# xxayt/MGSV

Hardware: AMD Instinct MI355X
Metric: video-music pairs/s fwd+bwd at B=64 (full training step); sub-objects: retrieval sim-matrix GB/s, eval forward pairs/s (higher is better)
Workload: dtype bf16; 1 GPU; BASELINE.json configs[2]: B=64/GPU, T_v=30, T_a=512, D=512, train mode (dropout on), f32 master weights + Adam, f32 gradient accumulation; global_batch=64, launch=tape

## Files before the change

mgsv_amd/csrc/linear.hip:

```cpp
#include "common.h"

namespace {

constexpr int BM = 128, BN = 128;
constexpr int KB = 128;
constexpr int LDS_ROW = KB + 16;
constexpr int NTHREADS = 256;

template <typename TC> struct Frag;
template <> struct Frag<float>  { typedef f32x4  type; };
template <> struct Frag<bf16_t> { typedef bf16x8 type; };

template <typename TC>
__device__ __forceinline__ typename Frag<TC>::type zero_frag() {
    typename Frag<TC>::type z;
#pragma unroll
    for (int i = 0; i < elem_traits<TC>::per16; ++i) z[i] = (TC)0.f;
    return z;
}

template <typename TA, typename TC>
__device__ __forceinline__ typename Frag<TC>::type load_a_frag(const TA* __restrict__ p, const TA* __restrict__ p2) {
    constexpr int n = elem_traits<TC>::per16;
    float v[n];
// ... 339 lines not shown
                SplitF32x4 sa[2][2], sw2[2][2];
#pragma unroll
                for (int u = 0; u < 2; ++u)
#pragma unroll
                    for (int t = 0; t < 2; ++t) {
                        sa[u][t] = made_split4(*(const f32x4*)(la + t * 32 * LDS_ROW + (ks + u) * 32));
                        sw2[u][t] = made_split4(*(const f32x4*)(lw + t * 32 * LDS_ROW + (ks + u) * 32));
                    }
#pragma unroll
                for (int mt = 0; mt < 2; ++mt)
#pragma unroll
                    for (int nt = 0; nt < 2; ++nt)
                        acc[mt][nt] = transposed ? made_mfma_x3_16(sw2[0][nt], sw2[1][nt], sa[0][mt], sa[1][mt], acc[mt][nt])
                                                 : made_mfma_x3_16(sa[0][mt], sa[1][mt], sw2[0][nt], sw2[1][nt], acc[mt][nt]);
            }
        } else {
#pragma unroll
        for (int ks = 0; ks < 4; ++ks) {
            frag_t fa[2], fw[2];
#pragma unroll
            for (int t = 0; t < 2; ++t) {
                fa[t] = *(const frag_t*)(la + t * 32 * LDS_ROW + ks * 32);
                fw[t] = *(const frag_t*)(lw + t * 32 * LDS_ROW + ks * 32);
            }
#pragma unroll
            for (int mt = 0; mt < 2; ++mt)
#pragma unroll
                for (int nt = 0; nt < 2; ++nt) {
                    if constexpr (sizeof(TC) == 2) {
                        if (transposed)
                            acc[mt][nt] = __builtin_amdgcn_mfma_f32_32x32x16_bf16(fw[nt], fa[mt], acc[mt][nt], 0, 0, 0);
                        else
                            acc[mt][nt] = __builtin_amdgcn_mfma_f32_32x32x16_bf16(fa[mt], fw[nt], acc[mt][nt], 0, 0, 0);
                    } else {
#pragma unroll
                        for (int e = 0; e < 4; ++e) {
                            if (transposed)
                                acc[mt][nt] = __builtin_amdgcn_mfma_f32_32x32x2f32(fw[nt][e], fa[mt][e], acc[mt][nt], 0, 0, 0);
                            else
                                acc[mt][nt] = __builtin_amdgcn_mfma_f32_32x32x2f32(fa[mt][e], fw[nt][e], acc[mt][nt], 0, 0, 0);
                        }
                    }
                }
        }
        }
        if (kt + 1 < nk) store_stage(lds + ((kt + 1) & 1) * STAGE);
        __syncthreads();
    }

    float* Ct = (float*)lds;
#pragma unroll
    for (int mt = 0; mt < 2; ++mt)
#pragma unroll
        for (int nt = 0; nt < 2; ++nt)
#pragma unroll
            for (int e = 0; e < 16; ++e) {
                int row, col;
                if (transposed) { row = wn * 64 + nt * 32 + acc_row(e, hh); col = wm * 64 + mt * 32 + r; }
                else            { row = wm * 64 + mt * 32 + acc_row(e, hh); col = wn * 64 + nt * 32 + r; }
                Ct[row * CT_LD + col] = acc[mt][nt][e];
            }
    __syncthreads();

    if (splitk > 1) {
        float* wsp = a.split_ws + (int64_t)blockIdx.z * M * N;
        const int cc = tid & 15;
        const int n = n0 + cc * 8;
        const bool vec = (N % 4 == 0);
        for (int i = 0; i < 8; ++i) {
            const int row = (tid >> 4) + 16 * i;
            const int m = m0 + row;
            if (m >= M) break;
            const float* cp = Ct + row * CT_LD + cc * 8;
            if (vec && n + 8 <= N) {
                *(f32x4*)(wsp + (int64_t)m * N + n) = *(const f32x4*)cp;
                *(f32x4*)(wsp + (int64_t)m * N + n + 4) = *(const f32x4*)(cp + 4);
            } else {
                for (int j = 0; j < 8 && n + j < N; ++j) wsp[(int64_t)m * N + n + j] = cp[j];
            }
        }
        return;
    }
    unsigned char* outp = (unsigned char*)seg.out;
    const int64_t out_z = z * seg.out_z_stride;
    const int rpb = (int)seg.rows_per_batch, rmod = (int)a.r_row_mod;
    const int colb = (int)seg.col_begin;
    const int odt = seg.out_dtype;

    if (!transposed) {
        const int cc = tid & 15;
        const int n = n0 + cc * 8;
        int nvalid = N - n; nvalid = nvalid > 8 ? 8 : nvalid;
        if (nvalid > 0) {
            float bv[8];
            load_bias8(a.bias, n, N, bv);
            const bool out_vec = (seg.ldo % 8 == 0) && (seg.out_batch_stride % 8 == 0) && (seg.out_z_stride % 8 == 0) &&
                                 (((uintptr_t)outp & 15) == 0) && (colb % 8 == 0);
            const bool r_vec = a.R && (a.ldr % 8 == 0) && (((uintptr_t)a.R & 15) == 0);
#pragma unroll 2
            for (int i = 0; i < 8; ++i) {
                const int row = (tid >> 4) + 16 * i;
                const int ml = m0 + row;
                if (ml >= Mv) break;
                const int m = a.row_index ? a.row_index[ml] : ml;
                const float* cp = Ct + row * CT_LD + cc * 8;
                f32x4 c0 = *(const f32x4*)cp, c1 = *(const f32x4*)(cp + 4);
                float v[8] = {c0[0], c0[1], c0[2], c0[3], c1[0], c1[1], c1[2], c1[3]};
                epilogue8<true>(a, m, n, nvalid, v, bv, rmod, r_vec);
                int64_t orow;
                if (rpb > 0) {
                    const int b = m / rpb, t = m - b * rpb;
                    orow = (int64_t)b * seg.out_batch_stride + (int64_t)t * seg.ldo;
                } else {
                    orow = (int64_t)m * seg.ldo;
                }
                store8(outp, odt, out_z + orow + (n - colb), v, nvalid, out_vec);
            }
        }
    } else {
        const int col = tid & 127;
        const int m = m0 + col;
        if (m < M) {
            int64_t obase;
            if (rpb > 0) {
                const int b = m / rpb, t = m - b * rpb;
                obase = (int64_t)b * seg.out_batch_stride + t;
            } else {
                obase = m;
            }
            const bool zero = a.out_row_mask != nullptr && a.out_row_mask[m] == 0.f;
            const int rr = rmod > 0 ? m % rmod : m;
            for (int i = 0; i < 64; ++i) {
                const int row = (tid >> 7) + 2 * i;
                const int n = n0 + row;
                if (n >= N) break;
                float v = Ct[row * CT_LD + col];
                if (a.bias) v += a.bias[n];
                v = apply_act(v, a.act);
                if (a.R) v += load_as_f32(a.R, a.r_dtype, (int64_t)rr * a.ldr + n);
                if (zero) v = 0.f;
                store_from_f32(outp, odt, out_z + obase + (int64_t)(n - colb) * seg.ldo, v);
            }
        }
    }
}



constexpr int G_CT_LD = BN + 4;

__device__ __forceinline__ int swz(int row) { return (row >> 1) & 7; }

template <int NST, bool TRAIN, int BMT, typename TC = bf16_t, bool X3 = false>
__global__ __launch_bounds__(NTHREADS, NST == 1 ? (BMT == 64 ? 6 : (TRAIN ? 3 : 4)) : 1) void linear_glds_kernel(const MadeLinearArgs a) {
    constexpr int PER16 = 16 / (int)sizeof(TC), KE = KB / (int)sizeof(TC);
    constexpr int STAGE = (BMT + BN) * KB;
    constexpr int NT = BMT == 128 ? 2 : 1;
    constexpr int AP = BMT / 32;
    constexpr int EROWS = BMT == 128 ? 64 : 32;
    constexpr int CT_BYTES = EROWS * G_CT_LD * 4;
    __shared__ __attribute__((aligned(16))) unsigned char lds[NST == 1 ? (CT_BYTES > STAGE ? CT_BYTES : STAGE) : NST * STAGE];
    const int tid = threadIdx.x;
    const int lane = tid & 63, wave = tid >> 6;
    const int r = lane & 31, hh = lane >> 5;
    const int wm = BMT == 128 ? wave >> 1 : 0, wn = BMT == 128 ? wave & 1 : wave;

    const int M = (int)a.M, N = (int)a.N, K = (int)a.K;
    const int n_tiles = (N + BN - 1) / BN;
    int Mv = M;
    if (a.n_rows) { const int nv = *a.n_rows; Mv = nv < M ? nv : M; }
    const int nwg = ((Mv + BMT - 1) / BMT) * n_tiles;
    if ((int)blockIdx.x >= nwg) return;
    int tile_id;
    {
        const int xcd = blockIdx.x & 7, q = nwg >> 3, rem = nwg & 7;
        tile_id = (xcd < rem ? xcd * (q + 1) : rem * (q + 1) + (xcd - rem) * q) + (blockIdx.x >> 3);
    }
    const int tile_m = tile_id / n_tiles, tile_n = tile_id % n_tiles;
    const int m0 = tile_m * BMT, n0 = tile_n * BN;
    const int64_t z = blockIdx.z;

    int si = 0;
#pragma unroll
    for (int s = 1; s < 4; ++s)
        if (s < a.nseg && n0 >= a.seg[s].col_begin) si = s;
    const MadeLinearSeg seg = a.seg[si];


    if (a.tile_skip_mask) {
        const int g0 = m0 + lane, g1 = m0 + 64 + lane;
        const float v0 = g0 < M ? a.tile_skip_mask[g0] : 0.f, v1 = (BMT == 128 && g1 < M) ? a.tile_skip_mask[g1] : 0.f;
        if (!__any(v0 != 0.f || v1 != 0.f)) {
            if (a.out_row_mask && !seg.transposed && (a.split_k <= 1)) {
                const int rpb0 = (int)seg.rows_per_batch;
                for (int idx = tid; idx < BMT * (BN / 8); idx += NTHREADS) {
                    const int row = idx / (BN / 8), c8 = idx % (BN / 8);
                    const int m = m0 + row, n = n0 + c8 * 8;
                    if (m >= M || n >= N) continue;
                    int64_t orow;
                    if (rpb0 > 0) { const int b = m / rpb0, t = m - b * rpb0; orow = (int64_t)b * seg.out_batch_stride + (int64_t)t * seg.ldo; }
                    else orow = (int64_t)m * seg.ldo;
                    const float zero8[8] = {0.f, 0.f, 0.f, 0.f, 0.f, 0.f, 0.f, 0.f};
                    int nv = N - n; nv = nv > 8 ? 8 : nv;
                    store8(seg.out, seg.out_dtype, blockIdx.z * seg.out_z_stride + orow + (n - (int)seg.col_begin), zero8, nv, false);
                }
            }
            return;
        }
    }

    const TC* Abase = ((seg.use_a2 && a.A2 && a.a2_replace) ? (const TC*)a.A2 : (const TC*)a.A) + z * a.a_z_stride;
    const int64_t lda = (seg.use_a2 && a.A2 && a.a2_replace) ? a.lda2 : a.lda;
    const TC* Wbase = (const TC*)a.W + z * a.w_z_stride;
    const TC* pa[AP];
    const TC* pw[4];
#pragma unroll
    for (int i = 0; i < AP; ++i) {
        const int row = 8 * (AP * wave + i) + (lane >> 3);
        const int chunk = (lane & 7) ^ swz(row);
        int gm = m0 + row; gm = gm < Mv ? gm : Mv - 1;
        if (a.row_index) gm = a.row_index[gm];
        pa[i] = Abase + (int64_t)gm * lda + chunk * PER16;
    }
#pragma unroll
    for (int i = 0; i < 4; ++i) {
        const int row = 8 * (4 * wave + i) + (lane >> 3);
        const int chunk = (lane & 7) ^ swz(row);
        int gn = n0 + row; gn = gn < N ? gn : N - 1;
        pw[i] = Wbase + (int64_t)gn * a.ldw + chunk * PER16;
    }
    typedef __attribute__((address_space(3))) void* lds_ptr_t;
    typedef const __attribute__((address_space(1))) void* glb_ptr_t;

    f32x16 acc[2][NT];
#pragma unroll
    for (int i = 0; i < 2; ++i)
#pragma unroll
        for (int j = 0; j < NT; ++j)
#pragma unroll
            for (int e = 0; e < 16; ++e) acc[i][j][e] = 0.f;

    int offa[2], offw[NT], sa[2], sw[NT];
#pragma unroll
    for (int t = 0; t < 2; ++t) {
        const int ra = wm * 64 + t * 32 + r;
        offa[t] = ra * KB; sa[t] = swz(ra);
    }
#pragma unroll
    for (int t = 0; t < NT; ++t) {
        const int rw = wn * (NT * 32) + t * 32 + r;
        offw[t] = BMT * KB + rw * KB; sw[t] = swz(rw);
    }

    const int nk = K / KE;
    auto issue = [&](int kt, unsigned char* st) __attribute__((always_inline)) {
#pragma unroll
        for (int i = 0; i < AP; ++i)
            __builtin_amdgcn_global_load_lds((glb_ptr_t)(pa[i] + kt * KE), (lds_ptr_t)(st + (AP * wave + i) * 1024), 16, 0, 0);
#pragma unroll
        for (int i = 0; i < 4; ++i)
            __builtin_amdgcn_global_load_lds((glb_ptr_t)(pw[i] + kt * KE), (lds_ptr_t)(st + BMT * KB + (4 * wave + i) * 1024), 16, 0, 0);
    };
    auto multiply = [&](const unsigned char* st) __attribute__((always_inline)) {
        if constexpr (sizeof(TC) == 4 && X3) {
#pragma unroll
            for (int kq = 0; kq < 4; kq += 2) {
                SplitF32x4 sa2[2][2], sw2[2][NT];
#pragma unroll
                for (int u = 0; u < 2; ++u) {
                    const int c = 2 * (kq + u) + hh;
#pragma unroll
                    for (int t = 0; t < 2; ++t) sa2[u][t] = made_split4(*(const f32x4*)(st + offa[t] + ((c ^ sa[t]) << 4)));
#pragma unroll
                    for (int t = 0; t < NT; ++t) sw2[u][t] = made_split4(*(const f32x4*)(st + offw[t] + ((c ^ sw[t]) << 4)));
                }
#pragma unroll
                for (int mt = 0; mt < 2; ++mt)
#pragma unroll
                    for (int nt = 0; nt < NT; ++nt) acc[mt][nt] = made_mfma_x3_16(sa2[0][mt], sa2[1][mt], sw2[0][nt], sw2[1][nt], acc[mt][nt]);
            }
            return;
        }
        if constexpr (sizeof(TC) == 4) {
#pragma unroll
            for (int kq = 0; kq < 4; ++kq) {
                f32x4 fa[2], fw[NT];
                const int c = 2 * kq + hh;
#pragma unroll
                for (int t = 0; t < 2; ++t) fa[t] = *(const f32x4*)(st + offa[t] + ((c ^ sa[t]) << 4));
#pragma unroll
                for (int t = 0; t < NT; ++t) fw[t] = *(const f32x4*)(st + offw[t] + ((c ^ sw[t]) << 4));
#pragma unroll
                for (int j = 0; j < 4; ++j)
#pragma unroll
                    for (int mt = 0; mt < 2; ++mt)
#pragma unroll
                        for (int nt = 0; nt < NT; ++nt)
                            acc[mt][nt] = __builtin_amdgcn_mfma_f32_32x32x2f32(fa[mt][j], fw[nt][j], acc[mt][nt], 0, 0, 0);
            }
            return;
        }
#pragma unroll
        for (int ks = 0; ks < 4; ++ks) {
            bf16x8 fa[2], fw[NT];
            const int c = 2 * ks + hh;
#pragma unroll
            for (int t = 0; t < 2; ++t) fa[t] = *(const bf16x8*)(st + offa[t] + ((c ^ sa[t]) << 4));
#pragma unroll
            for (int t = 0; t < NT; ++t) fw[t] = *(const bf16x8*)(st + offw[t] + ((c ^ sw[t]) << 4));
#pragma unroll
            for (int mt = 0; mt < 2; ++mt)
#pragma unroll
                for (int nt = 0; nt < NT; ++nt)
                    acc[mt][nt] = __builtin_amdgcn_mfma_f32_32x32x16_bf16(fa[mt], fw[nt], acc[mt][nt], 0, 0, 0);
        }
    };
    if constexpr (NST == 1) {
        for (int kt = 0; kt < nk; ++kt) {
            issue(kt, lds);
            __syncthreads();
            multiply(lds);
            __syncthreads();
        }
    } else {
        static_assert(BMT == 128, "the multi-stage ring counts 8 loads per wave per slab");
        issue(0, lds);
        if (nk > 1) issue(1, lds + STAGE);
        for (int kt = 0; kt < nk; ++kt) {
            if (kt + 1 < nk) asm volatile("s_waitcnt vmcnt(8)" ::: "memory");
            else asm volatile("s_waitcnt vmcnt(0)" ::: "memory");
            asm volatile("s_waitcnt lgkmcnt(0)\n\ts_barrier" ::: "memory");
            if (kt + 2 < nk) issue(kt + 2, lds + ((kt + 2) % NST) * STAGE);
            multiply(lds + (kt % NST) * STAGE);
        }
        __syncthreads();
    }

    float* Ct = (float*)lds;
    unsigned char* outp = (unsigned char*)seg.out;
    const int64_t out_z = z * seg.out_z_stride;
    const int rpb = (int)seg.rows_per_batch, rmod = (int)a.r_row_mod;
    const int colb = (int)seg.col_begin;
    const int odt = seg.out_dtype;
    const int cc = tid & 15;
    const int n = n0 + cc * 8;
    int nvalid = N - n; nvalid = nvalid > 8 ? 8 : nvalid;
    float bv[8];
    load_bias8(a.bias, n, N, bv);
    const bool out_vec = (seg.ldo % 8 == 0) && (seg.out_batch_stride % 8 == 0) && (seg.out_z_stride % 8 == 0) &&
                         (((uintptr_t)outp & 15) == 0) && (colb % 8 == 0);
    const bool r_vec = a.R && (a.ldr % 8 == 0) && (((uintptr_t)a.R & 15) == 0);
#pragma unroll
    for (int half = 0; half < 2; ++half) {
        if (m0 + half * EROWS >= Mv) break;
        if constexpr (BMT == 128) {
            if (wm == half) {
#pragma unroll
                for (int mt = 0; mt < 2; ++mt)
#pragma unroll
                    for (int nt = 0; nt < 2; ++nt)
#pragma unroll
                        for (int e = 0; e < 16; ++e)
                            Ct[(mt * 32 + acc_row(e, hh)) * G_CT_LD + wn * 64 + nt * 32 + r] = acc[mt][nt][e];
            }
        } else {
#pragma unroll
            for (int e = 0; e < 16; ++e)
                Ct[acc_row(e, hh) * G_CT_LD + wn * 32 + r] = half == 0 ? acc[0][0][e] : acc[1][0][e];
        }
        __syncthreads();
        if (nvalid > 0) {
#pragma unroll 2
            for (int i = 0; i < EROWS / 16; ++i) {
                const int row = (tid >> 4) + 16 * i;
                const int ml = m0 + half * EROWS + row;
                if (ml >= Mv) break;
                const int m = a.row_index ? a.row_index[ml] : ml;
                const float* cp = Ct + row * G_CT_LD + cc * 8;
                f32x4 c0 = *(const f32x4*)cp, c1 = *(const f32x4*)(cp + 4);
                float v[8] = {c0[0], c0[1], c0[2], c0[3], c1[0], c1[1], c1[2], c1[3]};
                epilogue8<TRAIN>(a, m, n, nvalid, v, bv, rmod, r_vec);
                int64_t orow;
                if (rpb > 0) {
                    const int b = m / rpb, t = m - b * rpb;
                    orow = (int64_t)b * seg.out_batch_stride + (int64_t)t * seg.ldo;
                } else {
                    orow = (int64_t)m * seg.ldo;
                }
                store8(outp, odt, out_z + orow + (n - colb), v, nvalid, out_vec);
            }
        }
        __syncthreads();
    }
}

constexpr int BIG_BN = 256, BIG_THREADS = 512, BIG_NMAX = 2048;

__device__ __forceinline__ void big_load8(const void* p, int dt, int64_t off, float* v) {
    if (dt == MADE_BF16) {
        const bf16x8 t = *(const bf16x8*)((const bf16_t*)p + off);
#pragma unroll
        for (int j = 0; j < 8; ++j) v[j] = (float)t[j];
    } else {
        const f32x4 t0 = *(const f32x4*)((const float*)p + off), t1 = *(const f32x4*)((const float*)p + off + 4);
#pragma unroll
        for (int j = 0; j < 4; ++j) { v[j] = t0[j]; v[4 + j] = t1[j]; }
    }
}
__device__ __forceinline__ void big_store8(void* p, int dt, int64_t off, const float* v) {
    if (dt == MADE_BF16) {
        bf16x8 t;
#pragma unroll
        for (int j = 0; j < 8; ++j) t[j] = (bf16_t)v[j];
        *(bf16x8*)((bf16_t*)p + off) = t;
    } else {
        *(f32x4*)((float*)p + off) = (f32x4){v[0], v[1], v[2], v[3]};
        *(f32x4*)((float*)p + off + 4) = (f32x4){v[4], v[5], v[6], v[7]};
    }
}

template <int BMB, bool TRAIN, bool FAST>
__global__ __launch_bounds__(BIG_THREADS, 1) void linear_big_kernel(const MadeLinearArgs a) {
    constexpr int STAGE = (BMB + BIG_BN) * KB;
    constexpr int MT = BMB / 64;
    constexpr int PA = BMB / 64, PW = BIG_BN / 64;
    extern __shared__ __attribute__((aligned(16))) unsigned char blds[];
    float* bias_l = (float*)(blds + 2 * STAGE);
    const int tid = threadIdx.x;
    const int lane = tid & 63, wave = __builtin_amdgcn_readfirstlane(tid >> 6);
    const int r = lane & 31, hh = lane >> 5;
    const int wm = wave >> 2, wn = wave & 3;
    const int M = (int)a.M, N = (int)a.N, K = (int)a.K;
    const int n_tiles = (N + BIG_BN - 1) / BIG_BN;
    int Mv = M;
    if (a.n_rows) { const int nv = *a.n_rows; Mv = nv < M ? nv : M; }
    const int nwg = ((Mv + BMB - 1) / BMB) * n_tiles;
    const int G = (int)gridDim.x;
    const int bperm = ((int)blockIdx.x & 7) * (G >> 3) + ((int)blockIdx.x >> 3);
    if (bperm >= nwg) return;
    for (int i = tid; i < BIG_NMAX; i += BIG_THREADS) bias_l[i] = (a.bias && i < N) ? a.bias[i] : 0.f;

    typedef __attribute__((address_space(3))) void* lds_ptr_t;
    typedef const __attribute__((address_space(1))) void* glb_ptr_t;
    const int nk = K / 64;
    const int rmod = (int)a.r_row_mod;
    const bool r_vec = a.R && (a.ldr % 8 == 0) && (((uintptr_t)a.R & 15) == 0);
    const uint32_t drop_thr = made_drop_threshold(a.drop.p);
    const float drop_sc = 1.f / (1.f - a.drop.p);
    const uint64_t drop_seed = (TRAIN && FAST && a.drop.p > 0.f) ? made_drop_seed(a.drop) : 0;

    int offa[MT], offw[2], sa[MT], sw[2];
#pragma unroll
    for (int t = 0; t < MT; ++t) { const int ra = wm * (BMB / 2) + t * 32 + r; offa[t] = ra * KB; sa[t] = swz(ra); }
#pragma unroll
    for (int t = 0; t < 2; ++t) { const int rw = wn * 64 + t * 32 + r; offw[t] = BMB * KB + rw * KB; sw[t] = swz(rw); }

    const bf16_t* pa[PA];
    const bf16_t* pw[PW];
    auto tile_of = [&](int L, int& m0, int& n0) __attribute__((always_inline)) { m0 = (L / n_tiles) * BMB; n0 = (L % n_tiles) * BIG_BN; };
    auto seg_of = [&](int n0) __attribute__((always_inline)) {
        int si = 0;
#pragma unroll
        for (int s = 1; s < 4; ++s)
            if (s < a.nseg && n0 >= a.seg[s].col_begin) si = s;
        return si;
    };
    auto set_sources = [&](int m0, int n0) __attribute__((always_inline)) {
        const MadeLinearSeg& sg = a.seg[seg_of(n0)];
        const bool repl = sg.use_a2 && a.A2 && a.a2_replace;
        const bf16_t* Abase = repl ? (const bf16_t*)a.A2 : (const bf16_t*)a.A;
        const int64_t lda = repl ? a.lda2 : a.lda;
#pragma unroll
        for (int i = 0; i < PA; ++i) {
            const int row = 8 * (PA * wave + i) + (lane >> 3);
            int gm = m0 + row; gm = gm < Mv ? gm : Mv - 1;
            if (a.row_index) gm = a.row_index[gm];
            pa[i] = Abase + (int64_t)gm * lda + (((lane & 7) ^ swz(row)) * 8);
        }
#pragma unroll
        for (int i = 0; i < PW; ++i) {
            const int row = 8 * (PW * wave + i) + (lane >> 3);
            int gn = n0 + row; gn = gn < N ? gn : N - 1;
            pw[i] = (const bf16_t*)a.W + (int64_t)gn * a.ldw + (((lane & 7) ^ swz(row)) * 8);
        }
    };
    auto issue = [&](int kt, int stage) __attribute__((always_inline)) {
// ... 395 lines not shown
    store8(outp, seg.out_dtype, out_z + orow + (n - colb), v, nvalid, out_vec);
}

template <bool TRAIN>
__global__ __launch_bounds__(NTHREADS) void linear_tiny_kernel(const MadeLinearArgs a) {
    __shared__ __attribute__((aligned(16))) float Ct[4 * T_BM * T_CT_LD];
    linear_tiny_body<TRAIN>(a, blockIdx.x, blockIdx.z, Ct);
}

constexpr int U_BM = 16, U_BN = 16, U_CT_LD = U_BN + 4;

template <bool TRAIN, int SPW>
__global__ __launch_bounds__(NTHREADS) void linear_t16_kernel(const MadeLinearArgs a) {
    __shared__ __attribute__((aligned(16))) float Ct[4 * U_BM * U_CT_LD];
    const int tid = threadIdx.x;
    const int lane = tid & 63, wave = __builtin_amdgcn_readfirstlane(tid >> 6);
    const int r16 = lane & 15, kq = lane >> 4;
    const int M = (int)a.M, N = (int)a.N, K = (int)a.K;
    const int n_tiles = (N + U_BN - 1) / U_BN, m_tiles = (M + U_BM - 1) / U_BM;
    int tile_m, tile_n;
    {
        const int bx = blockIdx.x;
        if ((n_tiles & 7) == 0) { const int j = bx >> 3; tile_m = j % m_tiles; tile_n = (j / m_tiles) * 8 + (bx & 7); }
        else { tile_m = bx % m_tiles; tile_n = bx / m_tiles; }
    }
    const int m0 = tile_m * U_BM, n0 = tile_n * U_BN;
    const int64_t z = blockIdx.z;
    int Mv = M;
    if (a.n_rows) { const int nv = *a.n_rows; Mv = nv < M ? nv : M; }
    if (m0 >= Mv) return;
    int si = 0;
#pragma unroll
    for (int s = 1; s < 4; ++s)
        if (s < a.nseg && n0 >= a.seg[s].col_begin) si = s;
    const MadeLinearSeg seg = a.seg[si];
    const bool repl = seg.use_a2 && a.A2 && a.a2_replace;
    const bf16_t* Abase = (repl ? (const bf16_t*)a.A2 : (const bf16_t*)a.A) + z * a.a_z_stride;
    const int64_t lda = repl ? a.lda2 : a.lda;
    const int steps = K / 32;
    int gm = m0 + r16; gm = gm < Mv ? gm : Mv - 1;
    if (a.row_index) gm = a.row_index[gm];
    int gn = n0 + r16; gn = gn < N ? gn : N - 1;
    const bf16_t* pa = Abase + (int64_t)gm * lda + kq * 8;
    const bf16_t* pw = (const bf16_t*)a.W + z * a.w_z_stride + (int64_t)gn * a.ldw + kq * 8;
    bf16x8 fa[SPW], fw[SPW];
#pragma unroll
    for (int i = 0; i < SPW; ++i) {
        int s = wave + 4 * i; s = s < steps ? s : steps - 1;
        fw[i] = *(const bf16x8*)(pw + s * 32);
        fa[i] = *(const bf16x8*)(pa + s * 32);
    }
    const int e_cc = tid & 1, e_row = (tid >> 1) & 15;
    const int e_n = n0 + e_cc * 8;
    int e_nvalid = N - e_n; e_nvalid = e_nvalid > 8 ? 8 : e_nvalid;
    const int e_ml = m0 + e_row;
    int e_m = e_ml < Mv ? e_ml : Mv - 1;
    if (a.row_index) e_m = a.row_index[e_m];
    float e_bv[8];
    load_bias8(a.bias_row_scale ? a.bias + z * a.bias_z_stride : a.bias, e_n, N, e_bv);
    float e_bsc = 1.f;
    if (a.bias_row_scale) e_bsc = a.bias_row_scale[(int64_t)e_m * a.batch + z];
    const int e_rmod = (int)a.r_row_mod;
    const bool e_rpref = a.R && a.r_dtype == MADE_BF16 && (a.ldr % 8 == 0) && (((uintptr_t)a.R & 15) == 0) && e_nvalid == 8;
    const bool e_gpref = TRAIN && a.gate != MADE_GATE_NONE && a.g_dtype == MADE_BF16 && (a.ldg % 8 == 0) && (((uintptr_t)a.G & 15) == 0) && e_nvalid == 8;
    bf16x8 e_r = {}, e_g = {};
    if (e_rpref) e_r = *(const bf16x8*)((const bf16_t*)a.R + (int64_t)(e_rmod > 0 ? e_m % e_rmod : e_m) * a.ldr + e_n);
    if constexpr (TRAIN) { if (e_gpref) e_g = *(const bf16x8*)((const bf16_t*)a.G + (int64_t)e_m * a.ldg + e_n); }
    float e_om = 1.f;
    if (a.out_row_mask) e_om = a.out_row_mask[e_m];
    uint64_t e_seed = 0;
    if constexpr (TRAIN) { if (a.drop.p > 0.f) e_seed = made_drop_seed(a.drop); }

    f32x4 acc;
    acc[0] = acc[1] = acc[2] = acc[3] = 0.f;
#pragma unroll
    for (int i = 0; i < SPW; ++i)
        if (wave + 4 * i < steps) acc = __builtin_amdgcn_mfma_f32_16x16x32_bf16(fa[i], fw[i], acc, 0, 0, 0);
    float* mine = Ct + wave * (U_BM * U_CT_LD);
#pragma unroll
    for (int e = 0; e < 4; ++e) mine[(kq * 4 + e) * U_CT_LD + r16] = acc[e];
    __syncthreads();
    if (tid >= 32) return;
    const int n = e_n, nvalid = e_nvalid;
    if (nvalid <= 0 || e_ml >= Mv) return;
    float v[8];
#pragma unroll
    for (int j = 0; j < 8; ++j) v[j] = 0.f;
#pragma unroll
    for (int w = 0; w < 4; ++w) {
        const float* cp = Ct + w * (U_BM * U_CT_LD) + e_row * U_CT_LD + e_cc * 8;
        const f32x4 c0 = *(const f32x4*)cp, c1 = *(const f32x4*)(cp + 4);
        v[0] += c0[0]; v[1] += c0[1]; v[2] += c0[2]; v[3] += c0[3];
        v[4] += c1[0]; v[5] += c1[1]; v[6] += c1[2]; v[7] += c1[3];
    }
    unsigned char* outp = (unsigned char*)seg.out;
    const int64_t out_z = z * seg.out_z_stride;
    const int rpb = (int)seg.rows_per_batch, rmod = (int)a.r_row_mod;
    const int colb = (int)seg.col_begin;
    const bool out_vec = (seg.ldo % 8 == 0) && (seg.out_batch_stride % 8 == 0) && (seg.out_z_stride % 8 == 0) &&
                         (((uintptr_t)outp & 15) == 0) && (colb % 8 == 0);
    const bool r_vec = a.R && (a.ldr % 8 == 0) && (((uintptr_t)a.R & 15) == 0);
    const int m = e_m;
    if (a.bias_row_scale) {
#pragma unroll
        for (int j = 0; j < 8; ++j) e_bv[j] *= e_bsc;
    }
    EpiPre pre;
    pre.has_r = e_rpref; pre.r = e_r; pre.has_g = e_gpref; pre.g = e_g; pre.has_om = true; pre.om = e_om;
    pre.has_seed = TRAIN && a.drop.p > 0.f; pre.seed = e_seed;
    epilogue8<TRAIN>(a, m, n, nvalid, v, e_bv, rmod, r_vec, pre);
    int64_t orow;
    if (rpb > 0) {
        const int b = m / rpb, t = m - b * rpb;
        orow = (int64_t)b * seg.out_batch_stride + (int64_t)t * seg.ldo;
    } else {
        orow = (int64_t)m * seg.ldo;
    }
    store8(outp, seg.out_dtype, out_z + orow + (n - colb), v, nvalid, out_vec);
}

template <bool TRAIN>
static void launch_t16(const MadeLinearArgs& a, hipStream_t st) {
    const int steps = (int)(a.K / 32), spw = (steps + 3) / 4;
    dim3 g((unsigned)(((a.M + U_BM - 1) / U_BM) * ((a.N + U_BN - 1) / U_BN)), 1, (unsigned)a.batch), block(NTHREADS);
    if (spw <= 1) hipLaunchKernelGGL((linear_t16_kernel<TRAIN, 1>), g, block, 0, st, a);
    else if (spw <= 2) hipLaunchKernelGGL((linear_t16_kernel<TRAIN, 2>), g, block, 0, st, a);
    else if (spw <= 4) hipLaunchKernelGGL((linear_t16_kernel<TRAIN, 4>), g, block, 0, st, a);
    else hipLaunchKernelGGL((linear_t16_kernel<TRAIN, 8>), g, block, 0, st, a);
}

}


static int tile_pref() {
    const char* e = made_variant_env("MADE_LINEAR_TILE");
    return e ? atoi(e) : 0;
}

static int64_t tiny_max() {
    const char* e = made_variant_env("MADE_TINY_MAX");
    return e ? (int64_t)atoll(e) : 1024;
}

static int64_t f32_glds_min() {
    const char* e = made_variant_env("MADE_LINEAR_F32_GLDS_MIN");
    return e ? (int64_t)atoll(e) : 1;
}

static int64_t big_train_min() {
    const char* e = made_variant_env("MADE_LINEAR_BIG_TRAIN");
    return e ? (int64_t)atoll(e) : 0;
}

static int64_t t16_max() {
    static const int64_t v = [] { const char* e = made_variant_env("MADE_T16_MAX"); return e ? (int64_t)atoll(e) : (int64_t)4096; }();
    return v;
}

static bool big_fast_epilogue(const MadeLinearArgs& a) {
    auto al = [](const void* p, int64_t ld, int dt) { return (((uintptr_t)p & 15) == 0) && ld % (dt == MADE_BF16 ? 8 : 4) == 0; };
    bool ok = (a.act == MADE_ACT_NONE || a.act == MADE_ACT_RELU) && a.N % 8 == 0 && (a.gate == MADE_GATE_NONE || a.gate == MADE_GATE_RELU_OUT);
    if (a.gate != MADE_GATE_NONE) ok = ok && al(a.G, a.ldg, a.g_dtype);
    if (a.Zout) ok = ok && al(a.Zout, a.ldz, a.z_dtype);
    if (a.R) ok = ok && al(a.R, a.ldr, a.r_dtype);
    if (a.drop.p > 0.f) ok = ok && a.drop_col_div <= 1;
    for (int s = 0; s < a.nseg; ++s)
        ok = ok && a.seg[s].rows_per_batch == 0 && a.seg[s].col_begin % 8 == 0 && al(a.seg[s].out, a.seg[s].ldo, a.seg[s].out_dtype);
    return ok;
}

static int pick_variant(const MadeLinearArgs& a) {
    if (a.w_dtype != MADE_BF16) {
        bool fast = a.a_dtype == MADE_F32 && a.K % 32 == 0 && a.a_row_mask == nullptr && a.split_k <= 1 && (a.A2 == nullptr || a.a2_replace) &&
                    ((uintptr_t)a.A % 16 == 0) && ((uintptr_t)a.W % 16 == 0) && (a.lda % 4 == 0) && (a.ldw % 4 == 0) && a.bias_row_scale == nullptr &&
                    made_variant_env("MADE_LINEAR_F32_GLDS_OFF") == nullptr;
        for (int s = 0; s < a.nseg; ++s) fast = fast && !a.seg[s].transposed;
        if (a.A2 && a.a2_replace) fast = fast && (a.a2_row_mod == 0) && (a.lda2 % 4 == 0) && ((uintptr_t)a.A2 % 16 == 0);
        if (a.batch > 1) fast = fast && (a.a_z_stride % 4 == 0) && (a.w_z_stride % 4 == 0);
        const int64_t tiles = ((a.M + BM - 1) / BM) * ((a.N + BN - 1) / BN);
        const int64_t tiles64 = ((a.M + 63) / 64) * ((a.N + BN - 1) / BN);
        if (fast && tiles64 * a.batch >= f32_glds_min()) {
            const int64_t live = a.row_index ? (tiles * a.batch * 9) / 16 : tiles * a.batch;
            return live > 1280 ? MADE_LINEAR_GLDS128_F32 : MADE_LINEAR_GLDS64_F32;
        }
        return MADE_LINEAR_GENERAL_F32;
    }
    bool fast = a.a_dtype == MADE_BF16 && a.K % 64 == 0 && a.a_row_mask == nullptr && a.split_k <= 1 &&
                (a.A2 == nullptr || a.a2_replace) && ((uintptr_t)a.A % 16 == 0) && (a.lda % 8 == 0);
    for (int s = 0; s < a.nseg; ++s) fast = fast && !a.seg[s].transposed;
    if (a.A2 && a.a2_replace) fast = fast && (a.a2_row_mod == 0) && (a.lda2 % 8 == 0);
    if (!fast) return a.a_dtype == MADE_F32 ? MADE_LINEAR_GENERAL_F32IN : MADE_LINEAR_GENERAL_BF16;
    const int64_t tiles = ((a.M + BM - 1) / BM) * ((a.N + BN - 1) / BN);
    const int64_t tiles64 = ((a.M + S_BM - 1) / S_BM) * ((a.N + S_BN - 1) / S_BN);
    const int64_t tiles32 = ((a.M + T_BM - 1) / T_BM) * ((a.N + T_BN - 1) / T_BN);
    if (a.M <= 64 && a.K >= 128 && a.K <= 1024 && a.K % 32 == 0 && a.tile_skip_mask == nullptr && tile_pref() != 1 && tile_pref() != 32 &&
        ((a.M + 15) / 16) * ((a.N + 15) / 16) * a.batch <= t16_max())
        return MADE_LINEAR_TINY16;
    if (tiles32 * a.batch <= tiny_max() && a.K <= 1024 && a.tile_skip_mask == nullptr && tile_pref() != 1) return MADE_LINEAR_TINY;
    if (tiles64 * a.batch <= 256 && a.tile_skip_mask == nullptr) return MADE_LINEAR_SKINNY;
    if (tiles * a.batch <= 256) return MADE_LINEAR_GLDS3;
    {
        const bool train_like = a.gate != MADE_GATE_NONE || a.Zout != nullptr || a.drop.p > 0.f;
        bool big_ok = a.batch == 1 && a.tile_skip_mask == nullptr && a.N <= BIG_NMAX && a.ldw % 8 == 0 && (!train_like || big_fast_epilogue(a));
        for (int s = 0; s < a.nseg; ++s) big_ok = big_ok && (a.seg[s].col_begin % BIG_BN == 0) && a.seg[s].out_z_stride == 0;
        if (big_ok) {
            if (tile_pref() == 512) return MADE_LINEAR_BIG256;
            if (tile_pref() == 256) return MADE_LINEAR_BIG128;
            const int64_t tiles256 = ((a.M + 255) / 256) * ((a.N + BIG_BN - 1) / BIG_BN);
            if (tile_pref() == 0 && !a.row_index && tiles256 >= 2 * 256) return MADE_LINEAR_BIG256;
            const int64_t tiles128 = ((a.M + 127) / 128) * ((a.N + BIG_BN - 1) / BIG_BN);
            const int64_t live128 = a.row_index ? (tiles128 * 9) / 16 : tiles128;
            if (tile_pref() == 0 && big_train_min() > 0 && a.N % BIG_BN == 0 && live128 >= big_train_min() && big_fast_epilogue(a)) return MADE_LINEAR_BIG128;
        }
    }
    const int64_t live = a.row_index ? (tiles * a.batch * 9) / 16 : tiles * a.batch;
    if (tile_pref() == 64) return MADE_LINEAR_GLDS64;
    if (tile_pref() == 128) return MADE_LINEAR_GLDS128;
    if (live > 1280) return MADE_LINEAR_GLDS128;
    if (!a.row_index) {
        const int64_t slots = 256 * 4, rounds = (live + slots - 1) / slots;
        if (live * 10 >= rounds * slots * 9) return MADE_LINEAR_GLDS128;
    }
    return MADE_LINEAR_GLDS64;
}

static int linear_validate(const MadeLinearArgs& a) {
    MADE_REQUIRE(a.A && a.W, "made_linear: null A or W");
    MADE_REQUIRE(a.M >= 0 && a.N > 0 && a.K > 0, "made_linear: bad dims M=%lld N=%lld K=%lld",
                 (long long)a.M, (long long)a.N, (long long)a.K);
    MADE_REQUIRE(a.nseg >= 1 && a.nseg <= 4, "made_linear: nseg=%d out of range", a.nseg);
    MADE_REQUIRE(a.batch >= 1 && a.batch <= 65535, "made_linear: batch=%lld out of range", (long long)a.batch);
    MADE_REQUIRE(a.w_dtype == MADE_F32 || a.w_dtype == MADE_BF16, "made_linear: bad w_dtype %d", a.w_dtype);
    MADE_UNSUPPORTED(!(a.a_dtype == MADE_BF16 && a.w_dtype == MADE_F32),
                     "made_linear: bf16 activations with f32 weights are not supported");
    const int per16 = a.w_dtype == MADE_F32 ? 4 : 8;
    const int a_align = a.a_dtype == MADE_F32 ? 4 : 8;
    MADE_UNSUPPORTED(a.K % per16 == 0, "made_linear: K=%lld must be a multiple of %d", (long long)a.K, per16);
    MADE_UNSUPPORTED(a.lda % a_align == 0 && a.ldw % per16 == 0 && ((uintptr_t)a.A % 16) == 0 && ((uintptr_t)a.W % 16) == 0,
                     "made_linear: A/W rows must be 16-byte aligned (lda=%lld ldw=%lld)", (long long)a.lda, (long long)a.ldw);
    if (a.A2)
        MADE_UNSUPPORTED(a.lda2 % a_align == 0 && ((uintptr_t)a.A2 % 16) == 0, "made_linear: A2 rows must be 16-byte aligned");
    if (a.batch > 1)
        MADE_UNSUPPORTED(a.a_z_stride % a_align == 0 && a.w_z_stride % per16 == 0, "made_linear: batch strides must keep 16-byte alignment");
    for (int s = 0; s < a.nseg; ++s) {
        MADE_REQUIRE(a.seg[s].out != nullptr, "made_linear: segment %d has null out", s);
        MADE_REQUIRE(a.seg[s].col_begin >= 0 && a.seg[s].col_begin < a.N, "made_linear: segment %d col_begin out of range", s);
        if (s > 0) {
            MADE_REQUIRE(a.seg[s].col_begin > a.seg[s - 1].col_begin, "made_linear: segments must be ascending");
            MADE_UNSUPPORTED(a.seg[s].col_begin % BN == 0, "made_linear: segment boundaries must be multiples of %d", BN);
        } else {
            MADE_REQUIRE(a.seg[0].col_begin == 0, "made_linear: first segment must start at column 0");
        }
    }
    MADE_REQUIRE((a.row_index == nullptr) == (a.n_rows == nullptr), "made_linear: row_index and n_rows come together");
    if (a.row_index) {
        MADE_UNSUPPORTED(a.split_k <= 1 && a.batch == 1, "made_linear: row gather is not available with split-K or batches");
        for (int s = 0; s < a.nseg; ++s)
            MADE_UNSUPPORTED(!a.seg[s].transposed, "made_linear: row gather is not available on transposed segments");
    }
    if (a.bias_row_scale) {
        MADE_REQUIRE(a.bias != nullptr, "made_linear: bias_row_scale without bias");
        MADE_UNSUPPORTED(pick_variant(a) == MADE_LINEAR_TINY || pick_variant(a) == MADE_LINEAR_TINY16, "made_linear: bias_row_scale is served by the tiny-M kernels only");
    }
    if (a.gate != MADE_GATE_NONE) MADE_REQUIRE(a.G != nullptr, "made_linear: gate without G");
    if (a.gate != MADE_GATE_NONE || a.Zout || a.drop.p > 0.f) {
        MADE_REQUIRE(a.drop.p >= 0.f && a.drop.p < 1.f, "made_linear: dropout p=%f out of [0,1)", (double)a.drop.p);
        MADE_UNSUPPORTED(a.split_k <= 1, "made_linear: gate / Zout / dropout are not available with split-K");
        for (int s = 0; s < a.nseg; ++s)
            MADE_UNSUPPORTED(!a.seg[s].transposed, "made_linear: gate / Zout / dropout are not available on transposed segments");
    }
    return MADE_OK;
}

extern "C" int made_linear(const MadeLinearArgs* args, void* stream) {
    MADE_REQUIRE(args != nullptr, "made_linear: null args");
    const MadeLinearArgs& a = *args;
    { const int rc = linear_validate(a); if (rc != MADE_OK) return rc; }
    if (a.M == 0) return MADE_OK;
    const int64_t tiles = ((a.M + BM - 1) / BM) * ((a.N + BN - 1) / BN);
    MADE_UNSUPPORTED(tiles < (1LL << 31), "made_linear: too many tiles");
    if (a.split_k > 1) {
        MADE_REQUIRE(a.split_ws != nullptr, "made_linear: split_k > 1 needs split_ws");
        MADE_UNSUPPORTED(a.batch == 1 && a.nseg == 1 && !a.seg[0].transposed && a.split_k <= 256,
                         "made_linear: split-K needs batch == 1, one plain segment and split_k <= 256");
    }
    dim3 grid((unsigned)tiles, 1, (unsigned)(a.split_k > 1 ? a.split_k : a.batch)), block(NTHREADS);
    hipStream_t st = (hipStream_t)stream;
    const bool train = a.gate != MADE_GATE_NONE || a.Zout != nullptr || a.drop.p > 0.f;
    switch (pick_variant(a)) {
        case MADE_LINEAR_TINY16:
            if (train) launch_t16<true>(a, st); else launch_t16<false>(a, st);
            break;
        case MADE_LINEAR_TINY: {
            dim3 g32((unsigned)(((a.M + T_BM - 1) / T_BM) * ((a.N + T_BN - 1) / T_BN)), 1, (unsigned)a.batch);
            if (train) hipLaunchKernelGGL((linear_tiny_kernel<true>), g32, block, 0, st, a);
            else hipLaunchKernelGGL((linear_tiny_kernel<false>), g32, block, 0, st, a);
            break;
        }
        case MADE_LINEAR_SKINNY: {
            dim3 g64((unsigned)(((a.M + S_BM - 1) / S_BM) * ((a.N + S_BN - 1) / S_BN)), 1, (unsigned)a.batch);
            if (train) hipLaunchKernelGGL((linear_skinny_kernel<true>), g64, block, 0, st, a);
            else hipLaunchKernelGGL((linear_skinny_kernel<false>), g64, block, 0, st, a);
            break;
        }
        case MADE_LINEAR_GLDS3:
            if (train) hipLaunchKernelGGL((linear_glds_kernel<3, true, 128>), grid, block, 0, st, a);
            else hipLaunchKernelGGL((linear_glds_kernel<3, false, 128>), grid, block, 0, st, a);
            break;
        case MADE_LINEAR_GLDS64: {
            dim3 g((unsigned)(((a.M + 63) / 64) * ((a.N + BN - 1) / BN)), 1, (unsigned)a.batch);
            if (train) hipLaunchKernelGGL((linear_glds_kernel<1, true, 64>), g, block, 0, st, a);
            else hipLaunchKernelGGL((linear_glds_kernel<1, false, 64>), g, block, 0, st, a);
            break;
        }
        case MADE_LINEAR_GLDS128:
            if (train) hipLaunchKernelGGL((linear_glds_kernel<1, true, 128>), grid, block, 0, st, a);
            else hipLaunchKernelGGL((linear_glds_kernel<1, false, 128>), grid, block, 0, st, a);
            break;
        case MADE_LINEAR_GLDS64_F32: {
            dim3 g((unsigned)(((a.M + 63) / 64) * ((a.N + BN - 1) / BN)), 1, (unsigned)a.batch);
            if (train) { if (g_made_f32_products) hipLaunchKernelGGL((linear_glds_kernel<1, true, 64, float, true>), g, block, 0, st, a); else hipLaunchKernelGGL((linear_glds_kernel<1, true, 64, float>), g, block, 0, st, a); }
            else { if (g_made_f32_products) hipLaunchKernelGGL((linear_glds_kernel<1, false, 64, float, true>), g, block, 0, st, a); else hipLaunchKernelGGL((linear_glds_kernel<1, false, 64, float>), g, block, 0, st, a); }
            break;
        }
        case MADE_LINEAR_GLDS128_F32:
            if (train) { if (g_made_f32_products) hipLaunchKernelGGL((linear_glds_kernel<1, true, 128, float, true>), grid, block, 0, st, a); else hipLaunchKernelGGL((linear_glds_kernel<1, true, 128, float>), grid, block, 0, st, a); }
            else { if (g_made_f32_products) hipLaunchKernelGGL((linear_glds_kernel<1, false, 128, float, true>), grid, block, 0, st, a); else hipLaunchKernelGGL((linear_glds_kernel<1, false, 128, float>), grid, block, 0, st, a); }
            break;
        case MADE_LINEAR_BIG256:
        case MADE_LINEAR_BIG128: {
            const bool b256 = pick_variant(a) == MADE_LINEAR_BIG256;
            const int bmb = b256 ? 256 : 128;
            const int ldsb = 2 * (bmb + BIG_BN) * KB + BIG_NMAX * 4;
            static const int n_cu = [] { int dev = 0, n = 0; (void)hipGetDevice(&dev); (void)hipDeviceGetAttribute(&n, hipDeviceAttributeMultiprocessorCount, dev); return n > 8 ? n : 256; }();
            static const bool once = [] {
                constexpr int l256 = 2 * (256 + BIG_BN) * KB + BIG_NMAX * 4, l128 = 2 * (128 + BIG_BN) * KB + BIG_NMAX * 4;
                bool ok = true;
                ok = ok && hipFuncSetAttribute((const void*)linear_big_kernel<256, false, false>, hipFuncAttributeMaxDynamicSharedMemorySize, l256) == hipSuccess;
                ok = ok && hipFuncSetAttribute((const void*)linear_big_kernel<256, false, true>, hipFuncAttributeMaxDynamicSharedMemorySize, l256) == hipSuccess;
                ok = ok && hipFuncSetAttribute((const void*)linear_big_kernel<128, false, false>, hipFuncAttributeMaxDynamicSharedMemorySize, l128) == hipSuccess;
                ok = ok && hipFuncSetAttribute((const void*)linear_big_kernel<128, false, true>, hipFuncAttributeMaxDynamicSharedMemorySize, l128) == hipSuccess;
                ok = ok && hipFuncSetAttribute((const void*)linear_big_kernel<256, true, true>, hipFuncAttributeMaxDynamicSharedMemorySize, l256) == hipSuccess;
                ok = ok && hipFuncSetAttribute((const void*)linear_big_kernel<128, true, true>, hipFuncAttributeMaxDynamicSharedMemorySize, l128) == hipSuccess;
                return ok;
            }();
            (void)once;
            const int64_t nt = ((a.M + bmb - 1) / bmb) * ((a.N + BIG_BN - 1) / BIG_BN);
            int64_t g = (n_cu / 8) * 8;
            if (nt < g) g = ((nt + 7) / 8) * 8;
            dim3 gb((unsigned)g), bb(BIG_THREADS);
            const bool fastep = big_fast_epilogue(a);
            const bool lite = fastep && (train || a.R != nullptr || a.out_row_mask != nullptr);
            if (b256) {
                if (lite) hipLaunchKernelGGL((linear_big_kernel<256, true, true>), gb, bb, ldsb, st, a);
                else if (fastep) hipLaunchKernelGGL((linear_big_kernel<256, false, true>), gb, bb, ldsb, st, a);
                else hipLaunchKernelGGL((linear_big_kernel<256, false, false>), gb, bb, ldsb, st, a);
            } else {
                if (lite) hipLaunchKernelGGL((linear_big_kernel<128, true, true>), gb, bb, ldsb, st, a);
                else if (fastep) hipLaunchKernelGGL((linear_big_kernel<128, false, true>), gb, bb, ldsb, st, a);
                else hipLaunchKernelGGL((linear_big_kernel<128, false, false>), gb, bb, ldsb, st, a);
            }
            break;
        }
        case MADE_LINEAR_GENERAL_F32IN: hipLaunchKernelGGL((linear_kernel<float, bf16_t>), grid, block, 0, st, a); break;
        case MADE_LINEAR_GENERAL_BF16: hipLaunchKernelGGL((linear_kernel<bf16_t, bf16_t>), grid, block, 0, st, a); break;
        default: if (g_made_f32_products) hipLaunchKernelGGL((linear_kernel<float, float, true>), grid, block, 0, st, a); else hipLaunchKernelGGL((linear_kernel<float, float>), grid, block, 0, st, a); break;
    }
    return made_check_launch("made_linear");
}

extern "C" int made_linear_variant(const MadeLinearArgs* args) {
    return args ? pick_variant(*args) : -1;
}
```

Before: 14040 pairs/s.

## Add multi-stage LDS ring pipeline for 64-row bf16 GEMM tiles

Extends the asynchronous global-to-LDS multi-stage ring, previously limited to 128-row tiles, to the 64-row GLDS kernel. The default is three stages, with a two-stage option behind an environment variable. Global addresses become a scalar base plus 32-bit per-lane offsets, and LDS fragment offsets are precomputed. The main loop now fetches all fragments into registers before issuing the next slab's loads and then runs the MFMAs, aiming to overlap memory latency with compute. The cost is more LDS per block and more registers, which lowers occupancy. Offsets are only used when the byte extent fits in 32 bits, and there is a new tile_pref override that forces the 64-row path.

```diff
diff --git a/mgsv_amd/csrc/linear.hip b/mgsv_amd/csrc/linear.hip
--- a/mgsv_amd/csrc/linear.hip
+++ b/mgsv_amd/csrc/linear.hip
@@ -515,7 +515,7 @@
 __device__ __forceinline__ int swz(int row) { return (row >> 1) & 7; }
 
 template <int NST, bool TRAIN, int BMT, typename TC = bf16_t, bool X3 = false>
-__global__ __launch_bounds__(NTHREADS, NST == 1 ? (BMT == 64 ? 6 : (TRAIN ? 3 : 4)) : 1) void linear_glds_kernel(const MadeLinearArgs a) {
+__global__ __launch_bounds__(NTHREADS, NST == 1 ? (BMT == 64 ? 6 : (TRAIN ? 3 : 4)) : (BMT == 128 ? 1 : (NST == 2 ? 3 : 2))) void linear_glds_kernel(const MadeLinearArgs a) {
     constexpr int PER16 = 16 / (int)sizeof(TC), KE = KB / (int)sizeof(TC);
     constexpr int STAGE = (BMT + BN) * KB;
     constexpr int NT = BMT == 128 ? 2 : 1;
@@ -575,8 +575,10 @@
     const TC* Abase = ((seg.use_a2 && a.A2 && a.a2_replace) ? (const TC*)a.A2 : (const TC*)a.A) + z * a.a_z_stride;
     const int64_t lda = (seg.use_a2 && a.A2 && a.a2_replace) ? a.lda2 : a.lda;
     const TC* Wbase = (const TC*)a.W + z * a.w_z_stride;
+    constexpr bool RING64 = NST > 1 && BMT == 64;
     const TC* pa[AP];
     const TC* pw[4];
+    unsigned va[AP], vw[4];
 #pragma unroll
     for (int i = 0; i < AP; ++i) {
         const int row = 8 * (AP * wave + i) + (lane >> 3);
@@ -584,6 +586,7 @@
         int gm = m0 + row; gm = gm < Mv ? gm : Mv - 1;
         if (a.row_index) gm = a.row_index[gm];
         pa[i] = Abase + (int64_t)gm * lda + chunk * PER16;
+        va[i] = (unsigned)(((int64_t)gm * lda + chunk * PER16) * (int64_t)sizeof(TC));
     }
 #pragma unroll
     for (int i = 0; i < 4; ++i) {
@@ -591,6 +594,7 @@
         const int chunk = (lane & 7) ^ swz(row);
         int gn = n0 + row; gn = gn < N ? gn : N - 1;
         pw[i] = Wbase + (int64_t)gn * a.ldw + chunk * PER16;
+        vw[i] = (unsigned)(((int64_t)gn * a.ldw + chunk * PER16) * (int64_t)sizeof(TC));
     }
     typedef __attribute__((address_space(3))) void* lds_ptr_t;
     typedef const __attribute__((address_space(1))) void* glb_ptr_t;
@@ -617,6 +621,20 @@
 
     const int nk = K / KE;
     auto issue = [&](int kt, unsigned char* st) __attribute__((always_inline)) {
+        if constexpr (RING64) {
+            const unsigned char* sa_k = (const unsigned char*)Abase + (int64_t)kt * KB;
+            const unsigned char* sw_k = (const unsigned char*)Wbase + (int64_t)kt * KB;
+            asm volatile("" : "+s"(sa_k));
+            asm volatile("" : "+s"(sw_k));
+            const int wu = __builtin_amdgcn_readfirstlane(wave);
+#pragma unroll
+            for (int i = 0; i < AP; ++i)
+                __builtin_amdgcn_global_load_lds((glb_ptr_t)(sa_k + va[i]), (lds_ptr_t)(st + (AP * wu + i) * 1024), 16, 0, 0);
+#pragma unroll
+            for (int i = 0; i < 4; ++i)
+                __builtin_amdgcn_global_load_lds((glb_ptr_t)(sw_k + vw[i]), (lds_ptr_t)(st + BMT * KB + (4 * wu + i) * 1024), 16, 0, 0);
+            return;
+        }
 #pragma unroll
         for (int i = 0; i < AP; ++i)
             __builtin_amdgcn_global_load_lds((glb_ptr_t)(pa[i] + kt * KE), (lds_ptr_t)(st + (AP * wave + i) * 1024), 16, 0, 0);
@@ -624,6 +642,18 @@
         for (int i = 0; i < 4; ++i)
             __builtin_amdgcn_global_load_lds((glb_ptr_t)(pw[i] + kt * KE), (lds_ptr_t)(st + BMT * KB + (4 * wave + i) * 1024), 16, 0, 0);
     };
+    constexpr bool HOIST = NST > 1 && sizeof(TC) == 2;
+    int foa[HOIST ? 4 : 1][2], fow[HOIST ? 4 : 1][NT];
+    if constexpr (HOIST) {
+#pragma unroll
+        for (int ks = 0; ks < 4; ++ks) {
+            const int c = 2 * ks + hh;
+#pragma unroll
+            for (int t = 0; t < 2; ++t) foa[ks][t] = offa[t] + ((c ^ sa[t]) << 4);
+#pragma unroll
+            for (int t = 0; t < NT; ++t) fow[ks][t] = offw[t] + ((c ^ sw[t]) << 4);
+        }
+    }
     auto multiply = [&](const unsigned char* st) __attribute__((always_inline)) {
         if constexpr (sizeof(TC) == 4 && X3) {
 #pragma unroll
@@ -676,6 +706,29 @@
 #pragma unroll
                 for (int nt = 0; nt < NT; ++nt)
                     acc[mt][nt] = __builtin_amdgcn_mfma_f32_32x32x16_bf16(fa[mt], fw[nt], acc[mt][nt], 0, 0, 0);
+        }
+    };
+    bf16x8 rfa[HOIST ? 4 : 1][2], rfw[HOIST ? 4 : 1][NT];
+    auto fetch = [&](const unsigned char* st) __attribute__((always_inline)) {
+        if constexpr (HOIST) {
+#pragma unroll
+            for (int ks = 0; ks < 4; ++ks) {
+#pragma unroll
+                for (int t = 0; t < 2; ++t) rfa[ks][t] = *(const bf16x8*)(st + foa[ks][t]);
+#pragma unroll
+                for (int t = 0; t < NT; ++t) rfw[ks][t] = *(const bf16x8*)(st + fow[ks][t]);
+            }
+        }
+    };
+    auto mma = [&]() __attribute__((always_inline)) {
+        if constexpr (HOIST) {
+#pragma unroll
+            for (int ks = 0; ks < 4; ++ks)
+#pragma unroll
+                for (int mt = 0; mt < 2; ++mt)
+#pragma unroll
+                    for (int nt = 0; nt < NT; ++nt)
+                        acc[mt][nt] = __builtin_amdgcn_mfma_f32_32x32x16_bf16(rfa[ks][mt], rfw[ks][nt], acc[mt][nt], 0, 0, 0);
         }
     };
     if constexpr (NST == 1) {
@@ -686,15 +739,25 @@
             __syncthreads();
         }
     } else {
-        static_assert(BMT == 128, "the multi-stage ring counts 8 loads per wave per slab");
-        issue(0, lds);
-        if (nk > 1) issue(1, lds + STAGE);
-        for (int kt = 0; kt < nk; ++kt) {
-            if (kt + 1 < nk) asm volatile("s_waitcnt vmcnt(8)" ::: "memory");
-            else asm volatile("s_waitcnt vmcnt(0)" ::: "memory");
-            asm volatile("s_waitcnt lgkmcnt(0)\n\ts_barrier" ::: "memory");
-            if (kt + 2 < nk) issue(kt + 2, lds + ((kt + 2) % NST) * STAGE);
-            multiply(lds + (kt % NST) * STAGE);
+        static_assert(sizeof(TC) == 2 && (NST == 3 || (NST == 2 && BMT == 64)), "the multi-stage rings: bf16, three stages, or two of 64 rows");
+        constexpr int LPS = AP + 4;
+#pragma unroll
+        for (int s = 0; s < NST - 1; ++s)
+            if (s < nk) issue(s, lds + s * STAGE);
+        for (int kt0 = 0; kt0 < nk; kt0 += NST) {
+#pragma unroll
+            for (int s = 0; s < NST; ++s) {
+                const int kt = kt0 + s;
+                if (kt >= nk) break;
+                if (NST == 3 && kt + 1 < nk) asm volatile("s_waitcnt vmcnt(%0)" ::"n"(LPS) : "memory");
+                else asm volatile("s_waitcnt vmcnt(0)" ::: "memory");
+                asm volatile("s_waitcnt lgkmcnt(0)\n\ts_barrier" ::: "memory");
+                fetch(lds + s * STAGE);
+                __builtin_amdgcn_sched_barrier(0);
+                if (kt + NST - 1 < nk) issue(kt + NST - 1, lds + ((s + NST - 1) % NST) * STAGE);
+                __builtin_amdgcn_sched_barrier(0);
+                mma();
+            }
         }
         __syncthreads();
     }
@@ -1396,6 +1459,16 @@
     return e ? (int64_t)atoll(e) : 0;
 }
 
+constexpr int RING64_DEFAULT = 3;
+static int ring64_stages(const MadeLinearArgs& a) {
+    const int64_t lda = (a.A2 && a.a2_replace) ? (a.lda2 > a.lda ? a.lda2 : a.lda) : a.lda;
+    const bool fits = ((a.M - 1) * lda + a.K) * 2 <= 0xffffffffLL && ((a.N - 1) * a.ldw + a.K) * 2 <= 0xffffffffLL;
+    if (a.K / 64 < 2 || !fits) return 0;
+    const char* e = made_variant_env("MADE_LINEAR_RING64");
+    const int v = e ? atoi(e) : RING64_DEFAULT;
+    return v == 2 || v == 3 ? v : 0;
+}
+
 static int64_t t16_max() {
     static const int64_t v = [] { const char* e = made_variant_env("MADE_T16_MAX"); return e ? (int64_t)atoll(e) : (int64_t)4096; }();
     return v;
@@ -1434,6 +1507,7 @@
     for (int s = 0; s < a.nseg; ++s) fast = fast && !a.seg[s].transposed;
     if (a.A2 && a.a2_replace) fast = fast && (a.a2_row_mod == 0) && (a.lda2 % 8 == 0);
     if (!fast) return a.a_dtype == MADE_F32 ? MADE_LINEAR_GENERAL_F32IN : MADE_LINEAR_GENERAL_BF16;
+    if (tile_pref() == -64) return MADE_LINEAR_GLDS64;
     const int64_t tiles = ((a.M + BM - 1) / BM) * ((a.N + BN - 1) / BN);
     const int64_t tiles64 = ((a.M + S_BM - 1) / S_BM) * ((a.N + S_BN - 1) / S_BN);
     const int64_t tiles32 = ((a.M + T_BM - 1) / T_BM) * ((a.N + T_BN - 1) / T_BN);
@@ -1553,7 +1627,14 @@
             break;
         case MADE_LINEAR_GLDS64: {
             dim3 g((unsigned)(((a.M + 63) / 64) * ((a.N + BN - 1) / BN)), 1, (unsigned)a.batch);
-            if (train) hipLaunchKernelGGL((linear_glds_kernel<1, true, 64>), g, block, 0, st, a);
+            const int ring = ring64_stages(a);
+            if (ring == 3) {
+                if (train) hipLaunchKernelGGL((linear_glds_kernel<3, true, 64>), g, block, 0, st, a);
+                else hipLaunchKernelGGL((linear_glds_kernel<3, false, 64>), g, block, 0, st, a);
+            } else if (ring == 2) {
+                if (train) hipLaunchKernelGGL((linear_glds_kernel<2, true, 64>), g, block, 0, st, a);
+                else hipLaunchKernelGGL((linear_glds_kernel<2, false, 64>), g, block, 0, st, a);
+            } else if (train) hipLaunchKernelGGL((linear_glds_kernel<1, true, 64>), g, block, 0, st, a);
             else hipLaunchKernelGGL((linear_glds_kernel<1, false, 64>), g, block, 0, st, a);
             break;
         }
```

Result: slower. 12820 pairs/s (-8.7%).
